# fakerlove1/HPFG

Measured on NVIDIA B200. Metric: UNet SSL train images/sec @224x224 (Mean-Teacher step), higher is better.
Workload: dtype bf16

## Files before the change

### hpfg_b200/csrc/tc_common.cuh

```cuda
#pragma once
#include <string>

#include "common.cuh"
#include "tc_ptx.cuh"

namespace hpfg {

constexpr int kTH = 16, kTW = 8;

__device__ __forceinline__ void unpack8(const uint4 &v, float (&f)[8]) {
    const uint32_t w[4] = {v.x, v.y, v.z, v.w};
#pragma unroll
    for (int i = 0; i < 4; ++i) {
        f[2 * i] = __uint_as_float(w[i] << 16);
        f[2 * i + 1] = __uint_as_float(w[i] & 0xffff0000u);
    }
}
__device__ __forceinline__ uint32_t pack2(float a, float b) {
    const __nv_bfloat162 h = __floats2bfloat162_rn(a, b);
    return *reinterpret_cast<const uint32_t *>(&h);
}

struct TileIter {
    int n_img, th, tw, dn, dh, dw;
    __device__ __forceinline__ void init(int mt, int step, int tiles_h, int tiles_w) {
        const int tpi = tiles_h * tiles_w;
        n_img = mt / tpi;
        int r = mt % tpi;
        th = r / tiles_w;
        tw = r % tiles_w;
        dn = step / tpi;
        r = step % tpi;
        dh = r / tiles_w;
        dw = r % tiles_w;
    }
    __device__ __forceinline__ void next(int tiles_h, int tiles_w) {
        tw += dw;
        if (tw >= tiles_w) { tw -= tiles_w; ++th; }
        th += dh;
        if (th >= tiles_h) { th -= tiles_h; ++n_img; }
        n_img += dn;
    }
};

typedef CUresult (*EncodeTiledFn)(CUtensorMap *, CUtensorMapDataType, cuuint32_t, void *, const cuuint64_t *, const cuuint64_t *,
                                  const cuuint32_t *, const cuuint32_t *, CUtensorMapInterleave, CUtensorMapSwizzle,
                                  CUtensorMapL2promotion, CUtensorMapFloatOOBfill);
inline EncodeTiledFn get_encode() {
    static EncodeTiledFn fn = nullptr;
    if (!fn) {
        void *p = nullptr;
        cudaDriverEntryPointQueryResult qres;
        if (cudaGetDriverEntryPoint("cuTensorMapEncodeTiled", &p, cudaEnableDefault, &qres) == cudaSuccess &&
            qres == cudaDriverEntryPointSuccess)
            fn = reinterpret_cast<EncodeTiledFn>(p);
    }
    return fn;
}

inline int make_map(CUtensorMap *m, const void *base, int N, int H, int W, int Cc, int kc, int box_w, int box_h) {
    EncodeTiledFn enc = get_encode();
    if (!enc) {
        set_error("cuTensorMapEncodeTiled entry point not available");
        return HPFG_ERR_CUDA;
    }
    cuuint64_t dims[4] = {(cuuint64_t)Cc, (cuuint64_t)W, (cuuint64_t)H, (cuuint64_t)N};
    cuuint64_t strides[3] = {(cuuint64_t)Cc * 2, (cuuint64_t)W * Cc * 2, (cuuint64_t)H * W * Cc * 2};
    cuuint32_t box[4] = {(cuuint32_t)kc, (cuuint32_t)box_w, (cuuint32_t)box_h, 1};
    cuuint32_t estr[4] = {1, 1, 1, 1};
    CUresult r = enc(m, CU_TENSOR_MAP_DATA_TYPE_BFLOAT16, 4, const_cast<void *>(base), dims, strides, box, estr,
                     CU_TENSOR_MAP_INTERLEAVE_NONE, CU_TENSOR_MAP_SWIZZLE_NONE, CU_TENSOR_MAP_L2_PROMOTION_L2_128B,
                     CU_TENSOR_MAP_FLOAT_OOB_FILL_NONE);
    if (r != CUDA_SUCCESS) {
        set_error("cuTensorMapEncodeTiled failed with code " + std::to_string((int)r));
        return HPFG_ERR_CUDA;
    }
    return HPFG_OK;
}


inline int make_map_chunked(CUtensorMap *m, const void *base, int N, int H, int W, int Cc, int chunks, int box_w, int box_h) {
    EncodeTiledFn enc = get_encode();
    if (!enc) {
        set_error("cuTensorMapEncodeTiled entry point not available");
        return HPFG_ERR_CUDA;
    }
    cuuint64_t dims[5] = {8, (cuuint64_t)W, (cuuint64_t)H, (cuuint64_t)(Cc / 8), (cuuint64_t)N};
    cuuint64_t strides[4] = {(cuuint64_t)Cc * 2, (cuuint64_t)W * Cc * 2, 16, (cuuint64_t)H * W * Cc * 2};
    cuuint32_t box[5] = {8, (cuuint32_t)box_w, (cuuint32_t)box_h, (cuuint32_t)chunks, 1};
    cuuint32_t estr[5] = {1, 1, 1, 1, 1};
    CUresult r = enc(m, CU_TENSOR_MAP_DATA_TYPE_BFLOAT16, 5, const_cast<void *>(base), dims, strides, box, estr,
                     CU_TENSOR_MAP_INTERLEAVE_NONE, CU_TENSOR_MAP_SWIZZLE_NONE, CU_TENSOR_MAP_L2_PROMOTION_L2_128B,
                     CU_TENSOR_MAP_FLOAT_OOB_FILL_NONE);
    if (r != CUDA_SUCCESS) {
        set_error("cuTensorMapEncodeTiled (chunked 5-D) failed with code " + std::to_string((int)r));
        return HPFG_ERR_CUDA;
    }
    return HPFG_OK;
}

}
```

### hpfg_b200/csrc/tc_ptx.cuh

```cuda
#pragma once
#include <cuda.h>
#include <cuda_runtime.h>
#include <cstdint>
#include <cstdio>

namespace hpfg {
namespace ptx {

__device__ __forceinline__ uint32_t smem_u32(const void *p) { return static_cast<uint32_t>(__cvta_generic_to_shared(p)); }

__device__ __forceinline__ void mbar_init(uint32_t bar, uint32_t count) {
    asm volatile("mbarrier.init.shared::cta.b64 [%0], %1;" ::"r"(bar), "r"(count) : "memory");
}
__device__ __forceinline__ void fence_barrier_init() { asm volatile("fence.mbarrier_init.release.cluster;" ::: "memory"); }
__device__ __forceinline__ void mbar_expect_tx(uint32_t bar, uint32_t bytes) {
    asm volatile("mbarrier.arrive.expect_tx.shared::cta.b64 _, [%0], %1;" ::"r"(bar), "r"(bytes) : "memory");
}
__device__ __forceinline__ void mbar_arrive(uint32_t bar) {
    asm volatile("mbarrier.arrive.shared::cta.b64 _, [%0];" ::"r"(bar) : "memory");
}
__device__ __forceinline__ bool mbar_try_wait(uint32_t bar, uint32_t parity) {
    uint32_t ok;
    asm volatile(
        "{\n\t.reg .pred p;\n\t"
        "mbarrier.try_wait.parity.shared::cta.b64 p, [%1], %2;\n\t"
        "selp.u32 %0, 1, 0, p;\n\t}"
        : "=r"(ok)
        : "r"(bar), "r"(parity)
        : "memory");
    return ok != 0;
}
__device__ __forceinline__ void mbar_wait(uint32_t bar, uint32_t parity, int tag) {
    if (mbar_try_wait(bar, parity)) return;
    const long long t0 = clock64();
    while (!mbar_try_wait(bar, parity)) {
        if (clock64() - t0 > 6000000000LL) {
            printf("hpfg_b200: mbarrier wait timed out (tag %d, block %d, thread %d, parity %u)\n", tag, (int)blockIdx.x,
                   (int)threadIdx.x, parity);
            __trap();
        }
    }
}

__device__ __forceinline__ void mbar_wait_warp(uint32_t bar, uint32_t parity, int tag) {
    if ((threadIdx.x & 31) == 0) mbar_wait(bar, parity, tag);
    __syncwarp();
}

__device__ __forceinline__ void fence_proxy_async_smem() { asm volatile("fence.proxy.async.shared::cta;" ::: "memory"); }

__device__ __forceinline__ uint4 lds128(uint32_t addr) {
    uint4 v;
    asm volatile("ld.shared.v4.u32 {%0, %1, %2, %3}, [%4];" : "=r"(v.x), "=r"(v.y), "=r"(v.z), "=r"(v.w) : "r"(addr) : "memory");
    return v;
}
__device__ __forceinline__ void sts128(uint32_t addr, const uint4 &v) {
    asm volatile("st.shared.v4.u32 [%0], {%1, %2, %3, %4};" ::"r"(addr), "r"(v.x), "r"(v.y), "r"(v.z), "r"(v.w) : "memory");
}

__device__ __forceinline__ void tma_load_4d(uint32_t dst, const CUtensorMap *map, uint32_t bar, int c0, int c1, int c2, int c3) {
    asm volatile(
        "cp.async.bulk.tensor.4d.shared::cluster.global.mbarrier::complete_tx::bytes [%0], [%1, {%3, %4, %5, %6}], [%2];"
        ::"r"(dst), "l"(reinterpret_cast<uint64_t>(map)), "r"(bar), "r"(c0), "r"(c1), "r"(c2), "r"(c3)
        : "memory");
}
__device__ __forceinline__ void tma_load_5d(uint32_t dst, const CUtensorMap *map, uint32_t bar, int c0, int c1, int c2, int c3, int c4) {
    asm volatile(
        "cp.async.bulk.tensor.5d.shared::cluster.global.mbarrier::complete_tx::bytes [%0], [%1, {%3, %4, %5, %6, %7}], [%2];"
        ::"r"(dst), "l"(reinterpret_cast<uint64_t>(map)), "r"(bar), "r"(c0), "r"(c1), "r"(c2), "r"(c3), "r"(c4)
        : "memory");
}
__device__ __forceinline__ void bulk_load(uint32_t dst, const void *src, uint32_t bytes, uint32_t bar) {
    asm volatile("cp.async.bulk.shared::cluster.global.mbarrier::complete_tx::bytes [%0], [%1], %2, [%3];" ::"r"(dst),
                 "l"(reinterpret_cast<uint64_t>(src)), "r"(bytes), "r"(bar)
                 : "memory");
}
__device__ __forceinline__ void prefetch_tensormap(const CUtensorMap *map) {
    asm volatile("prefetch.tensormap [%0];" ::"l"(reinterpret_cast<uint64_t>(map)) : "memory");
}

__device__ __forceinline__ void tmem_alloc(uint32_t dst_smem, uint32_t ncols) {
    asm volatile("tcgen05.alloc.cta_group::1.sync.aligned.shared::cta.b32 [%0], %1;" ::"r"(dst_smem), "r"(ncols) : "memory");
    asm volatile("tcgen05.relinquish_alloc_permit.cta_group::1.sync.aligned;" ::: "memory");
}
__device__ __forceinline__ void tmem_dealloc(uint32_t taddr, uint32_t ncols) {
    asm volatile("tcgen05.dealloc.cta_group::1.sync.aligned.b32 %0, %1;" ::"r"(taddr), "r"(ncols) : "memory");
}
__device__ __forceinline__ void tc_fence_before() { asm volatile("tcgen05.fence::before_thread_sync;" ::: "memory"); }
__device__ __forceinline__ void tc_fence_after() { asm volatile("tcgen05.fence::after_thread_sync;" ::: "memory"); }

__device__ __forceinline__ void umma_bf16(uint32_t d_tmem, uint64_t adesc, uint64_t bdesc, uint32_t idesc, uint32_t accumulate) {
    asm volatile(
        "{\n\t.reg .pred p;\n\t"
        "setp.ne.b32 p, %4, 0;\n\t"
        "tcgen05.mma.cta_group::1.kind::f16 [%0], %1, %2, %3, p;\n\t}"
        ::"r"(d_tmem), "l"(adesc), "l"(bdesc), "r"(idesc), "r"(accumulate)
        : "memory");
}
__device__ __forceinline__ void umma_commit(uint32_t bar) {
    asm volatile("tcgen05.commit.cta_group::1.mbarrier::arrive::one.shared::cluster.b64 [%0];" ::"r"(bar) : "memory");
}
__device__ __forceinline__ void tmem_ld16(uint32_t taddr, uint32_t *r) {
    asm volatile(
        "tcgen05.ld.sync.aligned.32x32b.x16.b32 {%0, %1, %2, %3, %4, %5, %6, %7, %8, %9, %10, %11, %12, %13, %14, %15}, [%16];"
        : "=r"(r[0]), "=r"(r[1]), "=r"(r[2]), "=r"(r[3]), "=r"(r[4]), "=r"(r[5]), "=r"(r[6]), "=r"(r[7]), "=r"(r[8]),
          "=r"(r[9]), "=r"(r[10]), "=r"(r[11]), "=r"(r[12]), "=r"(r[13]), "=r"(r[14]), "=r"(r[15])
        : "r"(taddr)
        : "memory");
}
__device__ __forceinline__ void tmem_ld_wait() { asm volatile("tcgen05.wait::ld.sync.aligned;" ::: "memory"); }

__device__ __forceinline__ uint64_t umma_desc(uint32_t saddr, uint32_t lbo_bytes, uint32_t sbo_bytes) {
    uint64_t d = 0;
    d |= (uint64_t)((saddr >> 4) & 0x3FFFu);
    d |= (uint64_t)((lbo_bytes >> 4) & 0x3FFFu) << 16;
    d |= (uint64_t)((sbo_bytes >> 4) & 0x3FFFu) << 32;
    d |= (uint64_t)1 << 46;
    return d;
}
__host__ __device__ constexpr uint32_t umma_idesc_bf16(int M, int N, int a_mn_major, int b_mn_major) {
    return (1u << 4) | (1u << 7) | (1u << 10) | ((uint32_t)a_mn_major << 15) | ((uint32_t)b_mn_major << 16) |
           ((uint32_t)(N >> 3) << 17) | ((uint32_t)(M >> 4) << 24);
}

__device__ __forceinline__ bool elect_one() {
    uint32_t pred;
    asm volatile(
        "{\n\t.reg .pred P;\n\t"
        "elect.sync _|P, 0xffffffff;\n\t"
        "selp.u32 %0, 1, 0, P;\n\t}"
        : "=r"(pred));
    return pred != 0;
}

__device__ __forceinline__ void named_bar_sync(int id, int nthreads) {
    asm volatile("bar.sync %0, %1;" ::"r"(id), "r"(nthreads) : "memory");
}

}
}
```

### hpfg_b200/csrc/wgrad_tc.cu

```cuda
#include <algorithm>
#include <cstdlib>

#include "conv_ref.cuh"
#include "conv_tc.cuh"
#include "tc_common.cuh"

namespace hpfg {

constexpr int kWgXfThreads = 256;
constexpr int kWgThreads = 128 + kWgXfThreads + 128;
#ifndef HPFG_WG_SMEM_KB
#define HPFG_WG_SMEM_KB 198
#endif
constexpr int kWgSmemBudget = HPFG_WG_SMEM_KB * 1024;

template <int KS, int NB, int COB, int MT, bool TWO = false>
struct WgCfg {
    static constexpr int PAD = KS / 2, KK = KS * KS;
    static constexpr int TWP = kTW * MT, TPIX = kTH * TWP;
    static constexpr int HH = kTH + KS - 1, HW = TWP + KS - 1, NPIX_X = HH * HW;
    static constexpr int XR_CHS = NPIX_X * 16, XR_OP = (NB / 8) * XR_CHS;
    static constexpr int ROWP = TWP * 16;
    static constexpr int XC = HH * ROWP;
    static constexpr int X3_OP = KS * (NB / 8) * XC;
    static constexpr int D_CHS = TPIX * 16, D_OP = (COB / 8) * D_CHS;
    static constexpr int al(int v) { return (v + 127) / 128 * 128; }
    static constexpr int OFF_DOP = 0, OFF_DRAW = al(D_OP), OFF_XR = OFF_DRAW + (TWO ? al(D_OP) : 0), OFF_X3 = OFF_XR + al(XR_OP),
                         OFF_ONE = OFF_X3 + X3_OP;
    static constexpr int STAGE_BYTES = al(OFF_ONE + XC);
    static constexpr int MROWS = KS * NB;
    static constexpr int UM = MROWS + 8 <= 64 ? 64 : 128;
    static constexpr int TAIL_PAD = al((UM / 8 - MROWS / 8 - 1) * XC);
    static constexpr int FIXED_BYTES = 1024 + 5 * 256 * 4;
    static constexpr int STAGES_RAW = (kWgSmemBudget - FIXED_BYTES - TAIL_PAD) / STAGE_BYTES;
    static constexpr int STAGES = STAGES_RAW > 8 ? 8 : STAGES_RAW;
    static constexpr int SMEM_BYTES = STAGES * STAGE_BYTES + TAIL_PAD + FIXED_BYTES + 1024;
    static constexpr int ACC = KS * COB;
    static constexpr int TMEM_COLS = (ACC <= 32) ? 32 : (ACC <= 64) ? 64 : (ACC <= 128) ? 128 : (ACC <= 256) ? 256 : 512;
    static_assert(STAGES >= 2, "need at least a double buffer");
    static_assert(ACC <= 512 && MROWS + 8 <= 128, "accumulators exceed TMEM");
    static_assert(X3_OP % 128 == 0, "the ones group must start at the copies' group pitch");
};

struct WgParams {
    const float *scale, *shift;
    const float *dsc, *dkb, *dkd;
    const uint8_t *dropbits;
    float inv_keep;
    float *scratch;
    int N, H, W, Cin, Cout, tiles_h, tiles_w, m_tiles, ci_blocks, co_blocks, S;
    long long *trace;
};
#define WG_TRACE(role, idx) do { if (P.trace && blockIdx.x == 0 && lane == 0 && (idx) < 32) P.trace[(role) * 32 + (idx)] = clock64(); } while (0)

#ifndef HPFG_WG_MINBLOCKS
#define HPFG_WG_MINBLOCKS 2
#endif
template <int KS, int NB, int COB, int MT, bool TWO>
__global__ void __launch_bounds__(kWgThreads, HPFG_WG_MINBLOCKS) tc_wgrad_kernel(const __grid_constant__ CUtensorMap tmX,
                                                                 const __grid_constant__ CUtensorMap tmD,
                                                                 const __grid_constant__ CUtensorMap tmR, const WgParams P) {
    pdl_launch_dependents();
    using C = WgCfg<KS, NB, COB, MT, TWO>;
    extern __shared__ uint8_t smem_raw[];
    uint8_t *smem = reinterpret_cast<uint8_t *>((reinterpret_cast<uintptr_t>(smem_raw) + 1023) & ~uintptr_t(1023));
    uint8_t *fixed = smem + C::STAGES * C::STAGE_BYTES + C::TAIL_PAD;
    uint64_t *bars = reinterpret_cast<uint64_t *>(fixed);
    uint32_t *tmem_slot = reinterpret_cast<uint32_t *>(fixed + 512);
    float *s_scale = reinterpret_cast<float *>(fixed + 1024);
    float *s_shift = s_scale + 256;
    float *s_dsc = s_shift + 256, *s_dkb = s_dsc + 256, *s_dkd = s_dkb + 256;

    const int warp = __shfl_sync(0xffffffffu, (int)(threadIdx.x >> 5), 0), lane = threadIdx.x & 31;
    const uint32_t bar_full = ptx::smem_u32(bars), bar_xf = bar_full + 8 * C::STAGES, bar_empty = bar_xf + 8 * C::STAGES;
    const uint32_t bar_done = bar_empty + 8 * C::STAGES;
    const uint32_t smem_u32 = ptx::smem_u32(smem);

    const int n_bp = P.ci_blocks * P.co_blocks;
    const int bp = blockIdx.x % n_bp, split = blockIdx.x / n_bp;
    const int cib = bp % P.ci_blocks, cob = bp / P.ci_blocks;
    const int ci0 = cib * NB, co0 = cob * COB;
    const int n_work = (P.m_tiles - split + P.S - 1) / P.S;
    const bool xform = P.scale != nullptr, want_bias = cib == 0;

    if (threadIdx.x == 0) {
        for (int s = 0; s < C::STAGES; ++s) {
            ptx::mbar_init(bar_full + 8 * s, 1);
            ptx::mbar_init(bar_xf + 8 * s, kWgXfThreads / 32);
            ptx::mbar_init(bar_empty + 8 * s, 1);
        }
        ptx::mbar_init(bar_done, 1);
        ptx::fence_barrier_init();
        ptx::prefetch_tensormap(&tmX);
        ptx::prefetch_tensormap(&tmD);
        if (TWO) ptx::prefetch_tensormap(&tmR);
    }
    if (warp == 2) ptx::tmem_alloc(ptx::smem_u32(tmem_slot), C::TMEM_COLS);
    for (int i = threadIdx.x; i < C::STAGES * (C::XC / 16); i += blockDim.x)
        ptx::sts128(smem_u32 + (i / (C::XC / 16)) * C::STAGE_BYTES + C::OFF_ONE + (i % (C::XC / 16)) * 16, make_uint4(0x3f80u, 0u, 0u, 0u));
    ptx::fence_proxy_async_smem();
    pdl_wait();
    if (P.scale)
        for (int i = threadIdx.x; i < P.Cin; i += blockDim.x) { s_scale[i] = P.scale[i]; s_shift[i] = P.shift[i]; }
    if (TWO)
        for (int i = threadIdx.x; i < COB; i += blockDim.x) {
            const int co = co0 + i;
            const bool ok = co < P.Cout;
            s_dsc[i] = ok ? P.dsc[co] : 0.f; s_dkb[i] = ok ? P.dkb[co] : 0.f; s_dkd[i] = ok ? P.dkd[co] : 0.f;
        }
    ptx::tc_fence_before();
    __syncthreads();
    ptx::tc_fence_after();
    const uint32_t tmem_base = *tmem_slot;
    if (P.trace && blockIdx.x == 0 && threadIdx.x == 0) P.trace[5 * 32 + 2] = clock64();

    if (warp == 0) {
        TileIter ti;
        ti.init(split, P.S, P.tiles_h, P.tiles_w);
        int stage = 0, phase = 0;
#pragma unroll 1
        for (int it = 0; it < n_work; ++it) {
            const int h0 = ti.th * kTH, w0 = ti.tw * C::TWP;
            ptx::mbar_wait(bar_empty + 8 * stage, phase ^ 1, 11);
            WG_TRACE(0, it);
            const uint32_t sb = smem_u32 + stage * C::STAGE_BYTES;
            if (ptx::elect_one()) {
                ptx::mbar_expect_tx(bar_full + 8 * stage, C::D_OP * (TWO ? 2 : 1) + C::XR_OP);
                ptx::tma_load_5d(sb + C::OFF_DOP, &tmD, bar_full + 8 * stage, 0, w0, h0, co0 / 8, ti.n_img);
                if (TWO) ptx::tma_load_5d(sb + C::OFF_DRAW, &tmR, bar_full + 8 * stage, 0, w0, h0, co0 / 8, ti.n_img);
                ptx::tma_load_5d(sb + C::OFF_XR, &tmX, bar_full + 8 * stage, 0, w0 - C::PAD, h0 - C::PAD, ci0 / 8, ti.n_img);
            }
            __syncwarp();
            if (++stage == C::STAGES) { stage = 0; phase ^= 1; }
            ti.next(P.tiles_h, P.tiles_w);
        }
    } else if (warp == 1) {
        constexpr uint32_t idesc = ptx::umma_idesc_bf16(C::UM, COB, 1, 1);
        constexpr uint32_t a_hi = (uint32_t)(C::XC >> 4) | (1u << 14), b_hi = (uint32_t)(C::D_CHS >> 4) | (1u << 14);
        const uint32_t a_lo0 = (((smem_u32 + C::OFF_X3) >> 4) & 0x3FFFu) | ((uint32_t)(C::ROWP >> 4) << 16);
        const uint32_t b_lo0 = (((smem_u32 + C::OFF_DOP) >> 4) & 0x3FFFu) | ((uint32_t)(C::ROWP >> 4) << 16);
        int stage = 0, phase = 0;
#pragma unroll 1
        for (int it = 0; it < n_work; ++it) {
            ptx::mbar_wait(bar_xf + 8 * stage, phase, 14);
            ptx::tc_fence_after();
            WG_TRACE(3, it);
            const uint32_t a_lo = a_lo0 + stage * (C::STAGE_BYTES >> 4), b_lo = b_lo0 + stage * (C::STAGE_BYTES >> 4);
            if (ptx::elect_one()) {
#pragma unroll 2
                for (int j = 0; j < 8 * MT; ++j) {
                    const int jr = j / MT, jc = j % MT;
                    const uint64_t bd = ((uint64_t)b_hi << 32) | (uint64_t)(b_lo + (uint32_t)((2 * jr * C::ROWP + jc * 128) >> 4));
#pragma unroll
                    for (int r = 0; r < KS; ++r) {
                        const uint64_t ad = ((uint64_t)a_hi << 32) | (uint64_t)(a_lo + (uint32_t)(((2 * jr + r) * C::ROWP + jc * 128) >> 4));
                        ptx::umma_bf16(tmem_base + r * COB, ad, bd, idesc, (it == 0 && j == 0) ? 0u : 1u);
                    }
                }
                ptx::umma_commit(bar_empty + 8 * stage);
                if (it == n_work - 1) ptx::umma_commit(bar_done);
            }
            __syncwarp();
            WG_TRACE(4, it);
            if (++stage == C::STAGES) { stage = 0; phase ^= 1; }
        }
    } else if (warp >= 4 && warp < 4 + kWgXfThreads / 32) {
        const int t = threadIdx.x - 128;
        constexpr int NCHK = NB / 8, XPSTEP = kWgXfThreads / NCHK;
        const int xc = NCHK == 2 ? t % NCHK : t / XPSTEP, xp0 = NCHK == 2 ? t / NCHK : t % XPSTEP, xch = ci0 + xc * 8;
        float scl[8], shf[8];
#pragma unroll
        for (int k = 0; k < 8; ++k) { scl[k] = xform ? s_scale[xch + k] : 1.f; shf[k] = xform ? s_shift[xch + k] : 0.f; }
        TileIter ti;
        ti.init(split, P.S, P.tiles_h, P.tiles_w);
        int stage = 0, phase = 0;
#pragma unroll 1
        for (int it = 0; it < n_work; ++it) {
            const int h0 = ti.th * kTH - C::PAD, w0 = ti.tw * C::TWP - C::PAD;
            const size_t img_px = (size_t)ti.n_img * P.H;
            ptx::mbar_wait(bar_full + 8 * stage, phase, 15);
            if (warp == 4) WG_TRACE(1, it);
            const uint32_t sb = smem_u32 + stage * C::STAGE_BYTES;
            for (int p = xp0; p < C::NPIX_X; p += XPSTEP) {
                const int hr = p / C::HW, hc = p % C::HW;
                uint4 v = ptx::lds128(sb + C::OFF_XR + (xc * C::NPIX_X + p) * 16);
                if (xform) {
                    const int gh = h0 + hr, gw = w0 + hc;
                    if (gh >= 0 && gh < P.H && gw >= 0 && gw < P.W) {
                        float f[8];
                        unpack8(v, f);
                        uint32_t keep = 0xffu;
                        if (P.dropbits) keep = P.dropbits[(((img_px + gh) * P.W + gw) * P.Cin + xch) >> 3];
#pragma unroll
                        for (int k = 0; k < 8; ++k) {
                            float a = fmaf(f[k], scl[k], shf[k]);
                            a = fmaxf(a, kLeakySlope * a);
                            if (P.dropbits) a = ((keep >> k) & 1u) ? a * P.inv_keep : 0.f;
                            f[k] = a;
                        }
                        v = make_uint4(pack2(f[0], f[1]), pack2(f[2], f[3]), pack2(f[4], f[5]), pack2(f[6], f[7]));
                    } else {
                        v = make_uint4(0u, 0u, 0u, 0u);
                    }
                }
                const uint32_t dst = sb + C::OFF_X3 + xc * C::XC + (hr * C::TWP + hc) * 16;
#pragma unroll
                for (int s = 0; s < KS; ++s)
                    if (hc - s >= 0 && hc - s < C::TWP) ptx::sts128(dst + s * (NB / 8) * C::XC - s * 16, v);
            }
            if constexpr (TWO) {
                constexpr int NCD = COB / 8, GW = NCD >= 8 ? 1 : 8 / NCD;
                const int xw = warp - 4;
                const bool tile_border = h0 + C::PAD + kTH > P.H || w0 + C::PAD + C::TWP > P.W;
#pragma unroll 1
                for (int dc = NCD >= 8 ? xw : xw % NCD; dc < NCD; dc += 8) {
                    float a[8], b[8], d[8];
#pragma unroll
                    for (int k = 0; k < 8; ++k) { a[k] = s_dsc[dc * 8 + k]; b[k] = s_dkb[dc * 8 + k]; d[k] = s_dkd[dc * 8 + k]; }
#pragma unroll 2
                    for (int px = (NCD >= 8 ? 0 : (xw / NCD) * 32) + lane; px < C::TPIX; px += 32 * GW) {
                        const uint32_t addr = sb + C::OFF_DOP + (dc * C::TPIX + px) * 16;
                        float g[8], r[8];
                        unpack8(ptx::lds128(addr), g);
                        unpack8(ptx::lds128(addr + C::OFF_DRAW), r);
#pragma unroll
                        for (int k = 0; k < 8; ++k) g[k] = fmaf(a[k], g[k], fmaf(b[k], r[k], d[k]));
                        uint4 v = make_uint4(pack2(g[0], g[1]), pack2(g[2], g[3]), pack2(g[4], g[5]), pack2(g[6], g[7]));
                        if (tile_border) {
                            const int gh = h0 + C::PAD + px / C::TWP, gw = w0 + C::PAD + px % C::TWP;
                            if (gh >= P.H || gw >= P.W) v = make_uint4(0u, 0u, 0u, 0u);
                        }
                        ptx::sts128(addr, v);
                    }
                }
            }
            ptx::fence_proxy_async_smem();
            __syncwarp();
            if (lane == 0) ptx::mbar_arrive(bar_xf + 8 * stage);
            if (warp == 4) WG_TRACE(2, it);
            if (++stage == C::STAGES) { stage = 0; phase ^= 1; }
            ti.next(P.tiles_h, P.tiles_w);
        }
    } else if (warp >= 4 + kWgXfThreads / 32) {
        const int q = warp & 3;
        const int row = C::UM == 128 ? q * 32 + lane : (lane < 16 ? q * 16 + lane : C::MROWS);
        const int s_shift_idx = row / NB, ci = ci0 + row % NB;
        if (n_work > 0) {
            ptx::mbar_wait(bar_done, 0, 16);
            ptx::tc_fence_after();
            if (q == 0) WG_TRACE(5, 0);
            float *dst = P.scratch + (size_t)split * ((size_t)C::KK * P.Cin * P.Cout + P.Cout);
            if (want_bias) {
                const bool mine = C::UM == 128 ? (q * 32 + lane == C::MROWS) : (lane < 16 && q * 16 + lane == C::MROWS);
#pragma unroll 1
                for (int n0 = 0; n0 < COB; n0 += 16) {
                    uint32_t v[16];
                    ptx::tmem_ld16(tmem_base + ((uint32_t)(q * 32) << 16) + n0, v);
                    ptx::tmem_ld_wait();
                    if (mine) {
#pragma unroll
                        for (int jj = 0; jj < 16; ++jj)
                            if (co0 + n0 + jj < P.Cout) dst[(size_t)C::KK * P.Cin * P.Cout + co0 + n0 + jj] = __uint_as_float(v[jj]);
                    }
                }
            }
#pragma unroll 1
            for (int r = 0; r < KS; ++r) {
#pragma unroll 1
                for (int n0 = 0; n0 < COB; n0 += 16) {
                    uint32_t v[16];
                    ptx::tmem_ld16(tmem_base + ((uint32_t)(q * 32) << 16) + r * COB + n0, v);
                    ptx::tmem_ld_wait();
                    if (row < C::MROWS && ci < P.Cin) {
                        float *o = dst + ((size_t)(r * KS + s_shift_idx) * P.Cin + ci) * P.Cout + co0 + n0;
#pragma unroll
                        for (int jj = 0; jj < 16; jj += 4)
                            if (co0 + n0 + jj < P.Cout)
                                *reinterpret_cast<float4 *>(o + jj) = make_float4(__uint_as_float(v[jj]), __uint_as_float(v[jj + 1]),
                                                                                  __uint_as_float(v[jj + 2]), __uint_as_float(v[jj + 3]));
                    }
                }
            }
        }
    }
    ptx::tc_fence_before();
    __syncthreads();
    if (P.trace && blockIdx.x == 0 && threadIdx.x == 0) P.trace[5 * 32 + 1] = clock64();
    if (warp == 2) {
        ptx::tc_fence_after();
        ptx::tmem_dealloc(tmem_base, C::TMEM_COLS);
    }
}

__global__ void __launch_bounds__(256) tc_wgrad_reduce_kernel(const float *__restrict__ scratch, int S, int Cin, int Cout, int KK,
                                                              int cin_real, int cout_real, float *__restrict__ dw_oihw,
                                                              float *__restrict__ dbias, int accumulate) {
    pdl_prologue();
    __shared__ float part[8][32];
    const int64_t per = (int64_t)KK * Cin * Cout + Cout;
    const int ex = threadIdx.x & 31, g = threadIdx.x >> 5;
    const int64_t e = (int64_t)blockIdx.x * 32 + ex;
    float acc = 0.f;
    if (e < per) {
#pragma unroll 4
        for (int k = g; k < S; k += 8) acc += scratch[(int64_t)k * per + e];
    }
    part[g][ex] = acc;
    __syncthreads();
    if (g != 0 || e >= per) return;
    float s = 0.f;
#pragma unroll
    for (int k = 0; k < 8; ++k) s += part[k][ex];
    if (e < (int64_t)KK * Cin * Cout) {
        const int co = (int)(e % Cout), ci = (int)((e / Cout) % Cin), tap = (int)(e / ((int64_t)Cout * Cin));
        if (co < cout_real && ci < cin_real) {
            float *d = dw_oihw + ((int64_t)co * cin_real + ci) * KK + tap;
            *d = accumulate ? *d + s : s;
        }
    } else if (dbias && e - (int64_t)KK * Cin * Cout < cout_real) {
        float *d = dbias + (e - (int64_t)KK * Cin * Cout);
        *d = accumulate ? *d + s : s;
    }
}

static void wg_shape(int ks, int N, int H, int W, int Cin, int Cout, bool two, int &NB, int &COB, int &MT, int &ci_blocks, int &co_blocks, int &S,
                     int &m_tiles) {
    NB = Cin == 16 ? 16 : 32;
    COB = std::min(Cout, two ? 64 : 128);
    ci_blocks = Cin / NB;
    co_blocks = Cout / COB;
    MT = (ks == 3 && NB == 16 && COB <= 32 && W % (2 * kTW) == 0 && (int64_t)N * ((H + kTH - 1) / kTH) * (W / (2 * kTW)) >= 4 * kNumSMs) ? 2 : 1;
    m_tiles = N * ((H + kTH - 1) / kTH) * ((W + kTW * MT - 1) / (kTW * MT));
    S = std::max(1, std::min(tc_cta_cap(2) / (ci_blocks * co_blocks), m_tiles));
}

int64_t tc_wgrad_scratch_floats(int N, int H, int W, int Cin, int Cout, int KS) {
    int64_t need = 0;
    for (int two = 0; two < 2; ++two) {
        int NB, COB, MT, cib, cob, S, mt;
        wg_shape(KS, N, H, W, Cin, Cout, two != 0, NB, COB, MT, cib, cob, S, mt);
        need = std::max(need, (int64_t)S * ((int64_t)KS * KS * Cin * Cout + Cout));
    }
    return need;
}

template <int KS, int NB, int COB, int MT, bool TWO>
static int wg_launch(const CUtensorMap &mx, const CUtensorMap &md, const CUtensorMap &mr, const WgParams &P, cudaStream_t s) {
    using C = WgCfg<KS, NB, COB, MT, TWO>;
    static bool attr_set = false;
    if (!attr_set) {
        HPFG_CUDA_CHECK(cudaFuncSetAttribute(tc_wgrad_kernel<KS, NB, COB, MT, TWO>, cudaFuncAttributeMaxDynamicSharedMemorySize, C::SMEM_BYTES));
        attr_set = true;
    }
    const int grid = P.ci_blocks * P.co_blocks * P.S;
    HPFG_CUDA_CHECK(launch_pdl(tc_wgrad_kernel<KS, NB, COB, MT, TWO>, grid, kWgThreads, C::SMEM_BYTES, s, mx, md, mr, P));
    HPFG_LAUNCH_CHECK();
    return HPFG_OK;
}

template <int KS>
static int wg_dispatch(int NB, int COB, int MT, bool two, const CUtensorMap &mx, const CUtensorMap &md, const CUtensorMap &mr, const WgParams &P,
                       cudaStream_t s) {
#define HPFG_WG_CASE(nb, cob)                                                               \
    if (NB == nb && COB == cob) {                                                           \
        if constexpr (KS == 3 && cob <= 64) {        \
            if (two) {                                                                      \
                if constexpr (nb == 16 && cob <= 32) {                                      \
                    if (MT == 2) return wg_launch<KS, nb, cob, 2, true>(mx, md, mr, P, s);  \
                }                                                                           \
                return wg_launch<KS, nb, cob, 1, true>(mx, md, mr, P, s);                   \
            }                                                                               \
        }                                                                                   \
        if (two) break;                                                                     \
        if constexpr (KS == 3 && nb == 16 && cob <= 32) {                                   \
            if (MT == 2) return wg_launch<KS, nb, cob, 2, false>(mx, md, mr, P, s);         \
        }                                                                                   \
        return wg_launch<KS, nb, cob, 1, false>(mx, md, mr, P, s);                          \
    }
    do {
    HPFG_WG_CASE(16, 16) HPFG_WG_CASE(16, 32) HPFG_WG_CASE(16, 64) HPFG_WG_CASE(16, 128)
    HPFG_WG_CASE(32, 16) HPFG_WG_CASE(32, 32) HPFG_WG_CASE(32, 64) HPFG_WG_CASE(32, 128)
#undef HPFG_WG_CASE
    } while (0);
    set_error("tc wgrad: no kernel for NB=" + std::to_string(NB) + " COB=" + std::to_string(COB) + (two ? " (two-source dY)" : ""));
    return HPFG_ERR_UNSUPPORTED;
}

int tc_wgrad_run(int ks, int N, int H, int W, int Cin, int Cout, int cin_real, int cout_real, const void *x, LoadXform xf, const void *dy, float *scratch,
                 int64_t scratch_floats, float *dw_oihw, float *dbias, int accumulate, cudaStream_t s, const TcBwdFuse *fuse,
                 const TcWgradStreams *ws) {
    ProfScope _prof(PROF_WGRAD_TC, s);
    int NB, COB, MT;
    WgParams P{};
    const bool two = fuse && fuse->in_raw;
    wg_shape(ks, N, H, W, Cin, Cout, two, NB, COB, MT, P.ci_blocks, P.co_blocks, P.S, P.m_tiles);
    HPFG_REQUIRE(tc_wgrad_scratch_floats(N, H, W, Cin, Cout, ks) <= scratch_floats, "tc_wgrad: scratch too small");
    CUtensorMap mx, md, mr;
    HPFG_RETURN_IF(make_map_chunked(&mx, x, N, H, W, Cin, NB / 8, kTW * MT + ks - 1, kTH + ks - 1));
    HPFG_RETURN_IF(make_map_chunked(&md, dy, N, H, W, Cout, COB / 8, kTW * MT, kTH));
    mr = md;
    if (two) {
        HPFG_RETURN_IF(make_map_chunked(&mr, fuse->in_raw, N, H, W, Cout, COB / 8, kTW * MT, kTH));
        P.dsc = fuse->sc; P.dkb = fuse->kb; P.dkd = fuse->kd;
    }
    P.scale = xf.scale; P.shift = xf.shift;
    P.dropbits = reinterpret_cast<const uint8_t *>(xf.drop.bits); P.inv_keep = xf.drop.inv_keep;
    P.scratch = scratch;
    P.N = N; P.H = H; P.W = W; P.Cin = Cin; P.Cout = Cout;
    P.tiles_h = (H + kTH - 1) / kTH; P.tiles_w = (W + kTW * MT - 1) / (kTW * MT);
    static long long *trace_buf = nullptr;
    const bool want_trace = getenv("HPFG_WG_TRACE") != nullptr;
    if (want_trace && !trace_buf) cudaMalloc(&trace_buf, 6 * 32 * 8);
    if (want_trace) cudaMemsetAsync(trace_buf, 0, 6 * 32 * 8, s);
    P.trace = want_trace ? trace_buf : nullptr;
    HPFG_RETURN_IF(ks == 3 ? wg_dispatch<3>(NB, COB, MT, two, mx, md, mr, P, s) : wg_dispatch<1>(NB, COB, MT, two, mx, md, mr, P, s));
    if (want_trace && getenv("HPFG_WG_TRACE_DUMP")) {
        long long h[6 * 32];
        cudaStreamSynchronize(s);
        cudaMemcpy(h, trace_buf, sizeof(h), cudaMemcpyDeviceToHost);
        const long long t0 = h[5 * 32 + 2];
        const char *names[5] = {"tma:slot-free", "xf:tile-landed", "xf:done", "mma:operands-ready", "mma:issued"};
        printf("wgrad trace (CTA 0, cycles since setup): NB=%d COB=%d MT=%d S=%d grid=%d; epilogue starts %lld, kernel ends %lld\n", NB, COB, MT, P.S,
               P.ci_blocks * P.co_blocks * P.S, h[5 * 32] - t0, h[5 * 32 + 1] - t0);
        for (int r = 0; r < 5; ++r) {
            printf("%-20s", names[r]);
            for (int i = 0; i < 12; ++i) printf(" %6lld", h[r * 32 + i] ? h[r * 32 + i] - t0 : -1);
            printf("\n");
        }
        fflush(stdout);
    }
    const int64_t per = (int64_t)ks * ks * Cin * Cout + Cout;
    const int blocks = (int)((per + 31) / 32);
    if (ws && ws->reduce_stream) {
        HPFG_CUDA_CHECK(cudaEventRecord(ws->ev_partials, s));
        HPFG_CUDA_CHECK(cudaStreamWaitEvent(ws->reduce_stream, ws->ev_partials, 0));
        HPFG_CUDA_CHECK(launch_plain(tc_wgrad_reduce_kernel, blocks, 256, 0, ws->reduce_stream, (const float *)scratch, P.S, Cin, Cout, ks * ks, cin_real,
                                     cout_real, dw_oihw, dbias, accumulate));
        HPFG_LAUNCH_CHECK();
        HPFG_CUDA_CHECK(cudaEventRecord(ws->ev_reduced, ws->reduce_stream));
        return HPFG_OK;
    }
    HPFG_CUDA_CHECK(launch_pdl(tc_wgrad_reduce_kernel, blocks, 256, 0, s, scratch, P.S, Cin, Cout, ks * ks, cin_real, cout_real, dw_oihw, dbias, accumulate));
    HPFG_LAUNCH_CHECK();
    return HPFG_OK;
}

}

namespace hpfg {
template <int CMAX>
__global__ void __launch_bounds__(256) pad_to_nhwc16_kernel(const float *__restrict__ src, uint4 *__restrict__ dst, int N, int C, int H, int W, FastDiv dHW) {
    pdl_prologue();
    const uint32_t HW = dHW.d;
    const uint32_t total = (uint32_t)N * HW;
    for (uint32_t i = blockIdx.x * blockDim.x + threadIdx.x; i < total; i += gridDim.x * blockDim.x) {
        uint32_t n, pix;
        fast_divmod(i, dHW, n, pix);
        const float *sp = src + (size_t)n * C * HW + pix;
        float v[16];
#pragma unroll
        for (int c = 0; c < 16; ++c) v[c] = 0.f;
#pragma unroll
        for (int c = 0; c < CMAX; ++c)
            if (c < C) v[c] = __ldg(sp + (size_t)c * HW);
        dst[2 * (size_t)i] = make_uint4(pack2(v[0], v[1]), pack2(v[2], v[3]), pack2(v[4], v[5]), pack2(v[6], v[7]));
        dst[2 * (size_t)i + 1] = make_uint4(pack2(v[8], v[9]), pack2(v[10], v[11]), pack2(v[12], v[13]), pack2(v[14], v[15]));
    }
}
int pad_to_nhwc16(const float *src_nchw, void *dst, int N, int C, int H, int W, cudaStream_t s) {
    ProfScope _prof(PROF_GLUE, s);
    const int64_t total = (int64_t)N * H * W;
    const int blocks = (int)std::min<int64_t>((total + 255) / 256, (int64_t)kNumSMs * 16);
    if (C <= 4)
        HPFG_CUDA_CHECK(launch_pdl(pad_to_nhwc16_kernel<4>, blocks, 256, 0, s, src_nchw, reinterpret_cast<uint4 *>(dst), N, C, H, W, make_fastdiv((uint32_t)(H * W))));
    else
        HPFG_CUDA_CHECK(launch_pdl(pad_to_nhwc16_kernel<16>, blocks, 256, 0, s, src_nchw, reinterpret_cast<uint4 *>(dst), N, C, H, W, make_fastdiv((uint32_t)(H * W))));
    HPFG_LAUNCH_CHECK();
    return HPFG_OK;
}
}

using namespace hpfg;
extern "C" int hpfg_wgrad_tc_debug(int N, int H, int W, int cin, int cout, int ks, const void *x_bf16_nhwc,
                                   const void *dy_bf16_nhwc, const float *scale, const float *shift, float *dw_oihw,
                                   float *dbias, void *stream) {
    HPFG_REQUIRE(cin % 16 == 0 && cout % 16 == 0 && (ks == 1 || ks == 3), "hpfg_wgrad_tc_debug: unsupported shape");
    cudaStream_t s = (cudaStream_t)stream;
    const int64_t nf = tc_wgrad_scratch_floats(N, H, W, cin, cout, ks);
    float *scratch = nullptr;
    HPFG_CUDA_CHECK(cudaMalloc(&scratch, (size_t)nf * 4));
    LoadXform xf{};
    xf.scale = scale; xf.shift = shift; xf.drop.bits = nullptr; xf.drop.inv_keep = 1.f;
    const int rc = tc_wgrad_run(ks, N, H, W, cin, cout, cin, cout, x_bf16_nhwc, xf, dy_bf16_nhwc, scratch, nf, dw_oihw, dbias, 0, s, nullptr);
    cudaStreamSynchronize(s);
    cudaFree(scratch);
    if (rc == HPFG_OK) HPFG_CUDA_CHECK(cudaGetLastError());
    return rc;
}

extern "C" int hpfg_wgrad_tc_fused_debug(int N, int H, int W, int cin, int cout, int ks, const void *x_bf16_nhwc, const void *g_bf16_nhwc,
                                         const void *raw_bf16_nhwc, const float *sc, const float *kb, const float *kd, const float *scale,
                                         const float *shift, float *dw_oihw, float *dbias, void *stream) {
    HPFG_REQUIRE(cin % 16 == 0 && cout % 16 == 0 && ks == 3, "hpfg_wgrad_tc_fused_debug: unsupported shape");
    HPFG_REQUIRE(x_bf16_nhwc && g_bf16_nhwc && raw_bf16_nhwc && sc && kb && kd, "hpfg_wgrad_tc_fused_debug: null argument");
    cudaStream_t s = (cudaStream_t)stream;
    const int64_t nf = tc_wgrad_scratch_floats(N, H, W, cin, cout, ks);
    float *scratch = nullptr;
    HPFG_CUDA_CHECK(cudaMalloc(&scratch, (size_t)nf * 4));
    LoadXform xf{};
    xf.scale = scale; xf.shift = shift; xf.drop.bits = nullptr; xf.drop.inv_keep = 1.f;
    TcBwdFuse f;
    f.in_raw = raw_bf16_nhwc; f.sc = sc; f.kb = kb; f.kd = kd;
    const int rc = tc_wgrad_run(ks, N, H, W, cin, cout, cin, cout, x_bf16_nhwc, xf, g_bf16_nhwc, scratch, nf, dw_oihw, dbias, 0, s, &f);
    cudaStreamSynchronize(s);
    cudaFree(scratch);
    if (rc == HPFG_OK) HPFG_CUDA_CHECK(cudaGetLastError());
    return rc;
}

namespace hpfg {
int tc_run_bench(int op, int ks, int N, int H, int W, int cin, int cout, const void *in, void *out, const float *w, const float *scale,
                 const float *shift, float *stats, cudaStream_t s, int fuse_mode, const void *aux);
}
__global__ void fill_pattern_bf16(__nv_bfloat16 *p, size_t n, float scale) {
    pdl_prologue();
    for (size_t i = (size_t)blockIdx.x * blockDim.x + threadIdx.x; i < n; i += (size_t)gridDim.x * blockDim.x)
        p[i] = __float2bfloat16(scale * (float)((int)((i * 2654435761u) >> 24) - 128) / 128.f);
}
extern "C" int hpfg_conv_tc_bench(int op, int N, int H, int W, int cin, int cout, int ks, int iters, float *ms_out_host, void *stream) {
    HPFG_REQUIRE(op >= 0 && op <= 6 && iters > 0 && ms_out_host, "hpfg_conv_tc_bench: bad arguments");
    cudaStream_t s = (cudaStream_t)stream;
    const size_t px = (size_t)N * H * W;
    __nv_bfloat16 *a = nullptr, *b = nullptr, *aux = nullptr;
    float *w = nullptr, *sc = nullptr, *stats = nullptr, *scratch = nullptr, *dw = nullptr;
    const int64_t nf = tc_wgrad_scratch_floats(N, H, W, cin, cout, ks);
    HPFG_CUDA_CHECK(cudaMalloc(&a, px * std::max(cin, cout) * 2));
    HPFG_CUDA_CHECK(cudaMalloc(&b, px * std::max(cin, cout) * 2));
    HPFG_CUDA_CHECK(cudaMalloc(&aux, px * std::max(cin, cout) * 2));
    HPFG_CUDA_CHECK(cudaMemsetAsync(aux, 0, px * std::max(cin, cout) * 2, s));
    HPFG_CUDA_CHECK(cudaMalloc(&w, (size_t)cin * cout * ks * ks * 4));
    HPFG_CUDA_CHECK(cudaMalloc(&sc, 2 * 256 * 4));
    HPFG_CUDA_CHECK(cudaMalloc(&stats, (size_t)kNumSMs * 2 * 256 * 4 * 4));
    HPFG_CUDA_CHECK(cudaMalloc(&scratch, (size_t)nf * 4));
    HPFG_CUDA_CHECK(cudaMalloc(&dw, ((size_t)cin * cout * ks * ks + cout) * 4));
    HPFG_CUDA_CHECK(launch_pdl(fill_pattern_bf16, 1024, 256, 0, s, a, px * std::max(cin, cout), 1.f));
    HPFG_CUDA_CHECK(launch_pdl(fill_pattern_bf16, 1024, 256, 0, s, b, px * std::max(cin, cout), 1.f));
    HPFG_CUDA_CHECK(cudaMemsetAsync(w, 0, (size_t)cin * cout * ks * ks * 4, s));
    HPFG_CUDA_CHECK(cudaMemsetAsync(sc, 0, 2 * 256 * 4, s));
    cudaEvent_t e0, e1;
    cudaEventCreate(&e0);
    cudaEventCreate(&e1);
    LoadXform xf{};
    xf.scale = sc; xf.shift = sc + 256; xf.drop.bits = nullptr; xf.drop.inv_keep = 1.f;
    int rc = HPFG_OK;
    for (int i = -2; i < iters && rc == HPFG_OK; ++i) {
        if (i == 0) cudaEventRecord(e0, s);
        if (op == 2 || op == 6) {
            TcBwdFuse f;
            f.in_raw = aux; f.sc = sc; f.kb = sc; f.kd = sc;
            rc = tc_wgrad_run(ks, N, H, W, cin, cout, cin, cout, a, xf, b, scratch, nf, dw, dw + (size_t)cin * cout * ks * ks, 0, s, op == 6 ? &f : nullptr);
        } else if (op >= 3) {
            rc = tc_run_bench(1, ks, N, H, W, cin, cout, a, b, w, sc, sc + 256, stats, s, op - 2, aux);
        } else {
            rc = tc_run_bench(op, ks, N, H, W, cin, cout, a, b, w, op == 0 ? sc : nullptr, op == 0 ? sc + 256 : nullptr, op == 0 ? stats : nullptr, s, 0, nullptr);
        }
    }
    cudaEventRecord(e1, s);
    cudaStreamSynchronize(s);
    float ms = 0.f;
    cudaEventElapsedTime(&ms, e0, e1);
    *ms_out_host = ms / iters;
    cudaEventDestroy(e0); cudaEventDestroy(e1);
    cudaFree(a); cudaFree(b); cudaFree(aux); cudaFree(w); cudaFree(sc); cudaFree(stats); cudaFree(scratch); cudaFree(dw);
    if (rc == HPFG_OK) HPFG_CUDA_CHECK(cudaGetLastError());
    return rc;
}
```

Measured before the change: 10170.

## Decouple wgrad transformed-copy buffers from TMA ring and swizzle dY loads

Moves the transformed x-copy (A operand) buffers out of each TMA ring stage into a separate small set of NCP copy buffers with their own full/free mbarriers. This shrinks each ring stage, so more stages fit in shared memory and TMA can prefetch further ahead. For single-source, MT=1, COB multiple of 64, dY is loaded with 128B-swizzled 4-D TMA boxes and described to UMMA as SW128 K-major, in place of the chunked no-swizzle layout. The risks are extra barrier waits between the transform warps and the MMA warp, and getting the descriptor and offset math for the swizzled B operand right.

New measurement: 10270, median of 6. 1.01x the previous value.

```diff
diff --git a/hpfg_b200/csrc/tc_common.cuh b/hpfg_b200/csrc/tc_common.cuh
--- a/hpfg_b200/csrc/tc_common.cuh
+++ b/hpfg_b200/csrc/tc_common.cuh
@@ -58,7 +58,8 @@
     return fn;
 }
 
-inline int make_map(CUtensorMap *m, const void *base, int N, int H, int W, int Cc, int kc, int box_w, int box_h) {
+inline int make_map(CUtensorMap *m, const void *base, int N, int H, int W, int Cc, int kc, int box_w, int box_h,
+                    CUtensorMapSwizzle swizzle = CU_TENSOR_MAP_SWIZZLE_NONE) {
     EncodeTiledFn enc = get_encode();
     if (!enc) {
         set_error("cuTensorMapEncodeTiled entry point not available");
@@ -69,7 +70,7 @@
     cuuint32_t box[4] = {(cuuint32_t)kc, (cuuint32_t)box_w, (cuuint32_t)box_h, 1};
     cuuint32_t estr[4] = {1, 1, 1, 1};
     CUresult r = enc(m, CU_TENSOR_MAP_DATA_TYPE_BFLOAT16, 4, const_cast<void *>(base), dims, strides, box, estr,
-                     CU_TENSOR_MAP_INTERLEAVE_NONE, CU_TENSOR_MAP_SWIZZLE_NONE, CU_TENSOR_MAP_L2_PROMOTION_L2_128B,
+                     CU_TENSOR_MAP_INTERLEAVE_NONE, swizzle, CU_TENSOR_MAP_L2_PROMOTION_L2_128B,
                      CU_TENSOR_MAP_FLOAT_OOB_FILL_NONE);
     if (r != CUDA_SUCCESS) {
         set_error("cuTensorMapEncodeTiled failed with code " + std::to_string((int)r));
diff --git a/hpfg_b200/csrc/tc_ptx.cuh b/hpfg_b200/csrc/tc_ptx.cuh
--- a/hpfg_b200/csrc/tc_ptx.cuh
+++ b/hpfg_b200/csrc/tc_ptx.cuh
@@ -118,6 +118,7 @@
     d |= (uint64_t)1 << 46;
     return d;
 }
+constexpr uint32_t kUmmaLayoutSW128 = 2;
 __host__ __device__ constexpr uint32_t umma_idesc_bf16(int M, int N, int a_mn_major, int b_mn_major) {
     return (1u << 4) | (1u << 7) | (1u << 10) | ((uint32_t)a_mn_major << 15) | ((uint32_t)b_mn_major << 16) |
            ((uint32_t)(N >> 3) << 17) | ((uint32_t)(M >> 4) << 24);
diff --git a/hpfg_b200/csrc/wgrad_tc.cu b/hpfg_b200/csrc/wgrad_tc.cu
--- a/hpfg_b200/csrc/wgrad_tc.cu
+++ b/hpfg_b200/csrc/wgrad_tc.cu
@@ -13,6 +13,8 @@
 #define HPFG_WG_SMEM_KB 198
 #endif
 constexpr int kWgSmemBudget = HPFG_WG_SMEM_KB * 1024;
+
+constexpr bool wg_dy_sw128(int COB, int MT, bool TWO) { return !TWO && MT == 1 && COB % 64 == 0; }
 
 template <int KS, int NB, int COB, int MT, bool TWO = false>
 struct WgCfg {
@@ -24,23 +26,32 @@
     static constexpr int XC = HH * ROWP;
     static constexpr int X3_OP = KS * (NB / 8) * XC;
     static constexpr int D_CHS = TPIX * 16, D_OP = (COB / 8) * D_CHS;
+    static constexpr bool SW = wg_dy_sw128(COB, MT, TWO);
+    static constexpr int D_BOX = TPIX * 128;
     static constexpr int al(int v) { return (v + 127) / 128 * 128; }
-    static constexpr int OFF_DOP = 0, OFF_DRAW = al(D_OP), OFF_XR = OFF_DRAW + (TWO ? al(D_OP) : 0), OFF_X3 = OFF_XR + al(XR_OP),
-                         OFF_ONE = OFF_X3 + X3_OP;
-    static constexpr int STAGE_BYTES = al(OFF_ONE + XC);
+    static constexpr int alS(int v) { return SW ? (v + 1023) / 1024 * 1024 : al(v); }
+    static constexpr int CP_ONE = X3_OP, CP_BYTES = al(X3_OP + XC);
+    static constexpr int OFF_DOP = 0, OFF_DRAW = alS(D_OP), OFF_XR = OFF_DRAW + (TWO ? alS(D_OP) : 0);
+    static constexpr int STAGE_BYTES = alS(OFF_XR + XR_OP);
     static constexpr int MROWS = KS * NB;
     static constexpr int UM = MROWS + 8 <= 64 ? 64 : 128;
-    static constexpr int TAIL_PAD = al((UM / 8 - MROWS / 8 - 1) * XC);
     static constexpr int FIXED_BYTES = 1024 + 5 * 256 * 4;
-    static constexpr int STAGES_RAW = (kWgSmemBudget - FIXED_BYTES - TAIL_PAD) / STAGE_BYTES;
+    static constexpr int ring_slots(int ncp) { return (kWgSmemBudget - FIXED_BYTES - alS(ncp * CP_BYTES)) / STAGE_BYTES; }
+    static constexpr int NCP = ring_slots(4) >= 5 ? 4 : ring_slots(3) >= 4 ? 3 : 2;
+    static constexpr int RING_OFF = alS(NCP * CP_BYTES);
+    static constexpr int STAGES_RAW = (kWgSmemBudget - FIXED_BYTES - RING_OFF) / STAGE_BYTES;
     static constexpr int STAGES = STAGES_RAW > 8 ? 8 : STAGES_RAW;
-    static constexpr int SMEM_BYTES = STAGES * STAGE_BYTES + TAIL_PAD + FIXED_BYTES + 1024;
+    static constexpr int SMEM_BYTES = RING_OFF + STAGES * STAGE_BYTES + FIXED_BYTES + 1024;
     static constexpr int ACC = KS * COB;
     static constexpr int TMEM_COLS = (ACC <= 32) ? 32 : (ACC <= 64) ? 64 : (ACC <= 128) ? 128 : (ACC <= 256) ? 256 : 512;
     static_assert(STAGES >= 2, "need at least a double buffer");
     static_assert(ACC <= 512 && MROWS + 8 <= 128, "accumulators exceed TMEM");
     static_assert(X3_OP % 128 == 0, "the ones group must start at the copies' group pitch");
+    static_assert((NCP - 1) * CP_BYTES + (UM / 8) * XC <= RING_OFF + STAGES * STAGE_BYTES, "A-operand tail reads past the ring");
 };
+static_assert(WgCfg<3, 32, 128, 1>::STAGES == 3 && WgCfg<3, 32, 128, 1>::NCP == 2 && WgCfg<3, 32, 64, 1>::STAGES == 4 &&
+                  WgCfg<3, 32, 64, 1>::NCP == 2,
+              "weight-gradient ring depth differs from the plan");
 
 struct WgParams {
     const float *scale, *shift;
@@ -64,7 +75,7 @@
     using C = WgCfg<KS, NB, COB, MT, TWO>;
     extern __shared__ uint8_t smem_raw[];
     uint8_t *smem = reinterpret_cast<uint8_t *>((reinterpret_cast<uintptr_t>(smem_raw) + 1023) & ~uintptr_t(1023));
-    uint8_t *fixed = smem + C::STAGES * C::STAGE_BYTES + C::TAIL_PAD;
+    uint8_t *fixed = smem + C::RING_OFF + C::STAGES * C::STAGE_BYTES;
     uint64_t *bars = reinterpret_cast<uint64_t *>(fixed);
     uint32_t *tmem_slot = reinterpret_cast<uint32_t *>(fixed + 512);
     float *s_scale = reinterpret_cast<float *>(fixed + 1024);
@@ -72,9 +83,9 @@
     float *s_dsc = s_shift + 256, *s_dkb = s_dsc + 256, *s_dkd = s_dkb + 256;
 
     const int warp = __shfl_sync(0xffffffffu, (int)(threadIdx.x >> 5), 0), lane = threadIdx.x & 31;
-    const uint32_t bar_full = ptx::smem_u32(bars), bar_xf = bar_full + 8 * C::STAGES, bar_empty = bar_xf + 8 * C::STAGES;
-    const uint32_t bar_done = bar_empty + 8 * C::STAGES;
-    const uint32_t smem_u32 = ptx::smem_u32(smem);
+    const uint32_t bar_full = ptx::smem_u32(bars), bar_empty = bar_full + 8 * C::STAGES, bar_xf = bar_empty + 8 * C::STAGES;
+    const uint32_t bar_cfree = bar_xf + 8 * C::NCP, bar_done = bar_cfree + 8 * C::NCP;
+    const uint32_t smem_u32 = ptx::smem_u32(smem), ring_u32 = smem_u32 + C::RING_OFF;
 
     const int n_bp = P.ci_blocks * P.co_blocks;
     const int bp = blockIdx.x % n_bp, split = blockIdx.x / n_bp;
@@ -86,8 +97,11 @@
     if (threadIdx.x == 0) {
         for (int s = 0; s < C::STAGES; ++s) {
             ptx::mbar_init(bar_full + 8 * s, 1);
-            ptx::mbar_init(bar_xf + 8 * s, kWgXfThreads / 32);
             ptx::mbar_init(bar_empty + 8 * s, 1);
+        }
+        for (int b = 0; b < C::NCP; ++b) {
+            ptx::mbar_init(bar_xf + 8 * b, kWgXfThreads / 32);
+            ptx::mbar_init(bar_cfree + 8 * b, 1);
         }
         ptx::mbar_init(bar_done, 1);
         ptx::fence_barrier_init();
@@ -96,8 +110,8 @@
         if (TWO) ptx::prefetch_tensormap(&tmR);
     }
     if (warp == 2) ptx::tmem_alloc(ptx::smem_u32(tmem_slot), C::TMEM_COLS);
-    for (int i = threadIdx.x; i < C::STAGES * (C::XC / 16); i += blockDim.x)
-        ptx::sts128(smem_u32 + (i / (C::XC / 16)) * C::STAGE_BYTES + C::OFF_ONE + (i % (C::XC / 16)) * 16, make_uint4(0x3f80u, 0u, 0u, 0u));
+    for (int i = threadIdx.x; i < C::NCP * (C::XC / 16); i += blockDim.x)
+        ptx::sts128(smem_u32 + (i / (C::XC / 16)) * C::CP_BYTES + C::CP_ONE + (i % (C::XC / 16)) * 16, make_uint4(0x3f80u, 0u, 0u, 0u));
     ptx::fence_proxy_async_smem();
     pdl_wait();
     if (P.scale)
@@ -123,10 +137,16 @@
             const int h0 = ti.th * kTH, w0 = ti.tw * C::TWP;
             ptx::mbar_wait(bar_empty + 8 * stage, phase ^ 1, 11);
             WG_TRACE(0, it);
-            const uint32_t sb = smem_u32 + stage * C::STAGE_BYTES;
+            const uint32_t sb = ring_u32 + stage * C::STAGE_BYTES;
             if (ptx::elect_one()) {
                 ptx::mbar_expect_tx(bar_full + 8 * stage, C::D_OP * (TWO ? 2 : 1) + C::XR_OP);
-                ptx::tma_load_5d(sb + C::OFF_DOP, &tmD, bar_full + 8 * stage, 0, w0, h0, co0 / 8, ti.n_img);
+                if constexpr (C::SW) {
+#pragma unroll
+                    for (int b = 0; b < COB / 64; ++b)
+                        ptx::tma_load_4d(sb + C::OFF_DOP + b * C::D_BOX, &tmD, bar_full + 8 * stage, co0 + 64 * b, w0, h0, ti.n_img);
+                } else {
+                    ptx::tma_load_5d(sb + C::OFF_DOP, &tmD, bar_full + 8 * stage, 0, w0, h0, co0 / 8, ti.n_img);
+                }
                 if (TWO) ptx::tma_load_5d(sb + C::OFF_DRAW, &tmR, bar_full + 8 * stage, 0, w0, h0, co0 / 8, ti.n_img);
                 ptx::tma_load_5d(sb + C::OFF_XR, &tmX, bar_full + 8 * stage, 0, w0 - C::PAD, h0 - C::PAD, ci0 / 8, ti.n_img);
             }
@@ -136,21 +156,25 @@
         }
     } else if (warp == 1) {
         constexpr uint32_t idesc = ptx::umma_idesc_bf16(C::UM, COB, 1, 1);
-        constexpr uint32_t a_hi = (uint32_t)(C::XC >> 4) | (1u << 14), b_hi = (uint32_t)(C::D_CHS >> 4) | (1u << 14);
-        const uint32_t a_lo0 = (((smem_u32 + C::OFF_X3) >> 4) & 0x3FFFu) | ((uint32_t)(C::ROWP >> 4) << 16);
-        const uint32_t b_lo0 = (((smem_u32 + C::OFF_DOP) >> 4) & 0x3FFFu) | ((uint32_t)(C::ROWP >> 4) << 16);
+        constexpr uint32_t a_hi = (uint32_t)(C::XC >> 4) | (1u << 14);
+        constexpr uint32_t b_hi = C::SW ? (1024u >> 4) | (1u << 14) | (ptx::kUmmaLayoutSW128 << 29) : (uint32_t)(C::D_CHS >> 4) | (1u << 14);
+        constexpr uint32_t b_lbo = C::SW ? C::D_BOX : C::ROWP;
+        const uint32_t a_lo0 = ((smem_u32 >> 4) & 0x3FFFu) | ((uint32_t)(C::ROWP >> 4) << 16);
+        const uint32_t b_lo0 = (((ring_u32 + C::OFF_DOP) >> 4) & 0x3FFFu) | ((b_lbo >> 4) << 16);
         int stage = 0, phase = 0;
 #pragma unroll 1
         for (int it = 0; it < n_work; ++it) {
-            ptx::mbar_wait(bar_xf + 8 * stage, phase, 14);
+            const int cb = it % C::NCP, cphase = (it / C::NCP) & 1;
+            ptx::mbar_wait(bar_xf + 8 * cb, cphase, 14);
             ptx::tc_fence_after();
             WG_TRACE(3, it);
-            const uint32_t a_lo = a_lo0 + stage * (C::STAGE_BYTES >> 4), b_lo = b_lo0 + stage * (C::STAGE_BYTES >> 4);
+            const uint32_t a_lo = a_lo0 + cb * (C::CP_BYTES >> 4), b_lo = b_lo0 + stage * (C::STAGE_BYTES >> 4);
             if (ptx::elect_one()) {
 #pragma unroll 2
                 for (int j = 0; j < 8 * MT; ++j) {
                     const int jr = j / MT, jc = j % MT;
-                    const uint64_t bd = ((uint64_t)b_hi << 32) | (uint64_t)(b_lo + (uint32_t)((2 * jr * C::ROWP + jc * 128) >> 4));
+                    const uint32_t b_off = C::SW ? jr * 16 * 128 : 2 * jr * C::ROWP + jc * 128;
+                    const uint64_t bd = ((uint64_t)b_hi << 32) | (uint64_t)(b_lo + (b_off >> 4));
 #pragma unroll
                     for (int r = 0; r < KS; ++r) {
                         const uint64_t ad = ((uint64_t)a_hi << 32) | (uint64_t)(a_lo + (uint32_t)(((2 * jr + r) * C::ROWP + jc * 128) >> 4));
@@ -158,6 +182,7 @@
                     }
                 }
                 ptx::umma_commit(bar_empty + 8 * stage);
+                ptx::umma_commit(bar_cfree + 8 * cb);
                 if (it == n_work - 1) ptx::umma_commit(bar_done);
             }
             __syncwarp();
@@ -176,11 +201,13 @@
         int stage = 0, phase = 0;
 #pragma unroll 1
         for (int it = 0; it < n_work; ++it) {
+            const int cb = it % C::NCP, cphase = (it / C::NCP) & 1;
             const int h0 = ti.th * kTH - C::PAD, w0 = ti.tw * C::TWP - C::PAD;
             const size_t img_px = (size_t)ti.n_img * P.H;
             ptx::mbar_wait(bar_full + 8 * stage, phase, 15);
             if (warp == 4) WG_TRACE(1, it);
-            const uint32_t sb = smem_u32 + stage * C::STAGE_BYTES;
+            ptx::mbar_wait_warp(bar_cfree + 8 * cb, cphase ^ 1, 17);
+            const uint32_t sb = ring_u32 + stage * C::STAGE_BYTES, cbuf = smem_u32 + cb * C::CP_BYTES;
             for (int p = xp0; p < C::NPIX_X; p += XPSTEP) {
                 const int hr = p / C::HW, hc = p % C::HW;
                 uint4 v = ptx::lds128(sb + C::OFF_XR + (xc * C::NPIX_X + p) * 16);
@@ -203,7 +230,7 @@
                         v = make_uint4(0u, 0u, 0u, 0u);
                     }
                 }
-                const uint32_t dst = sb + C::OFF_X3 + xc * C::XC + (hr * C::TWP + hc) * 16;
+                const uint32_t dst = cbuf + xc * C::XC + (hr * C::TWP + hc) * 16;
 #pragma unroll
                 for (int s = 0; s < KS; ++s)
                     if (hc - s >= 0 && hc - s < C::TWP) ptx::sts128(dst + s * (NB / 8) * C::XC - s * 16, v);
@@ -236,7 +263,7 @@
             }
             ptx::fence_proxy_async_smem();
             __syncwarp();
-            if (lane == 0) ptx::mbar_arrive(bar_xf + 8 * stage);
+            if (lane == 0) ptx::mbar_arrive(bar_xf + 8 * cb);
             if (warp == 4) WG_TRACE(2, it);
             if (++stage == C::STAGES) { stage = 0; phase ^= 1; }
             ti.next(P.tiles_h, P.tiles_w);
@@ -344,9 +371,12 @@
     return need;
 }
 
+static int wg_last_stages = 0;
+
 template <int KS, int NB, int COB, int MT, bool TWO>
 static int wg_launch(const CUtensorMap &mx, const CUtensorMap &md, const CUtensorMap &mr, const WgParams &P, cudaStream_t s) {
     using C = WgCfg<KS, NB, COB, MT, TWO>;
+    wg_last_stages = C::STAGES;
     static bool attr_set = false;
     if (!attr_set) {
         HPFG_CUDA_CHECK(cudaFuncSetAttribute(tc_wgrad_kernel<KS, NB, COB, MT, TWO>, cudaFuncAttributeMaxDynamicSharedMemorySize, C::SMEM_BYTES));
@@ -397,7 +427,10 @@
     HPFG_REQUIRE(tc_wgrad_scratch_floats(N, H, W, Cin, Cout, ks) <= scratch_floats, "tc_wgrad: scratch too small");
     CUtensorMap mx, md, mr;
     HPFG_RETURN_IF(make_map_chunked(&mx, x, N, H, W, Cin, NB / 8, kTW * MT + ks - 1, kTH + ks - 1));
-    HPFG_RETURN_IF(make_map_chunked(&md, dy, N, H, W, Cout, COB / 8, kTW * MT, kTH));
+    if (wg_dy_sw128(COB, MT, two))
+        HPFG_RETURN_IF(make_map(&md, dy, N, H, W, Cout, 64, kTW, kTH, CU_TENSOR_MAP_SWIZZLE_128B));
+    else
+        HPFG_RETURN_IF(make_map_chunked(&md, dy, N, H, W, Cout, COB / 8, kTW * MT, kTH));
     mr = md;
     if (two) {
         HPFG_RETURN_IF(make_map_chunked(&mr, fuse->in_raw, N, H, W, Cout, COB / 8, kTW * MT, kTH));
@@ -420,8 +453,9 @@
         cudaMemcpy(h, trace_buf, sizeof(h), cudaMemcpyDeviceToHost);
         const long long t0 = h[5 * 32 + 2];
         const char *names[5] = {"tma:slot-free", "xf:tile-landed", "xf:done", "mma:operands-ready", "mma:issued"};
-        printf("wgrad trace (CTA 0, cycles since setup): NB=%d COB=%d MT=%d S=%d grid=%d; epilogue starts %lld, kernel ends %lld\n", NB, COB, MT, P.S,
-               P.ci_blocks * P.co_blocks * P.S, h[5 * 32] - t0, h[5 * 32 + 1] - t0);
+        printf("wgrad trace (CTA 0, cycles since setup): NB=%d COB=%d MT=%d S=%d grid=%d ring=%d dY=%s; epilogue starts %lld, kernel ends %lld\n", NB,
+               COB, MT, P.S, P.ci_blocks * P.co_blocks * P.S, wg_last_stages, wg_dy_sw128(COB, MT, two) ? "sw128" : "chunked", h[5 * 32] - t0,
+               h[5 * 32 + 1] - t0);
         for (int r = 0; r < 5; ++r) {
             printf("%-20s", names[r]);
             for (int i = 0; i < 12; ++i) printf(" %6lld", h[r * 32 + i] ? h[r * 32 + i] - t0 : -1);
```
